# xudoong/EdgeVisionTransformer

Measured on AMD Instinct MI355X. Metric: images/sec DeiT-base/16-224 bs=512 @1/2/4/8 GPU; % bf16 MFMA roofline, higher is better.
Workload: dtype bf16; 1 GPU; deit_base/16-224 forward, bs=512 per GPU, bf16; model=deit_base, global_batch=512, per_gpu_batch=512, seq_len=197, parallelism=dp1, gemm_variant=automatic, lanes=1

## Files before the change

edgevisiontransformer_amd/_lib.py:

```python
from __future__ import annotations

import ctypes
import os
import threading

import torch

_HERE = os.path.dirname(os.path.abspath(__file__))
LIB_PATH = os.environ.get("EVT_LIB", os.path.join(_HERE, "libevt_hip.so"))

EVT_OK = 0
EVT_EINVAL = -22
EVT_ENOMEM = -12
EVT_EHIP = -5
EVT_ENODEV = -19
DTYPE = {"f32": 0, "fp32": 0, "float32": 0, "bf16": 1, "bfloat16": 1, "mx8": 2}

EPI_BIAS, EPI_GELU, EPI_RESID, EPI_POS, EPI_OUT_F32 = 1, 2, 4, 8, 16
EPI_LNIN, EPI_RESLN, EPI_STATS, EPI_GELU_ERF = 32, 64, 128, 256
EPI_OUT_MX8 = 512
PROF_ROLES = ("patchify", "patch_embed", "qkv", "attention", "out_proj", "fc1", "fc2", "head",
              "(unused)", "t2t_unfold", "t2t_kqv", "t2t_performer", "merge", "attn_sublayer",
              "mlp")
SWIN_MAX_STAGES = 8
# ... 163 lines not shown

class evt_attn_args(ctypes.Structure):
    _fields_ = [("n_maps", ctypes.c_int32), ("blocks", ctypes.POINTER(ctypes.c_int32)),
                ("maps", ctypes.POINTER(ctypes.c_void_p)), ("queries", ctypes.c_int32)]


ATTN_CLS, ATTN_ALL = 0, 1
ATTENTION_SIGNATURES = {
    "evt_attn_map_shape": (_I, [_P, _I, _PI, _PI]),
    "evt_forward_attention": (_I, [_P, ctypes.POINTER(evt_image_args), _I,
                                   ctypes.POINTER(evt_features_args),
                                   ctypes.POINTER(evt_attn_args), _P]),
    "evt_attention_probs": (_I, [_I, _P, _I64, _I64, _I64, _I, _I, _I, _I, _I, _F, _I, _P, _P]),
}

_lib = None
_lock = threading.Lock()
_initialized_devices = set()


def load_library() -> ctypes.CDLL:
    global _lib
    with _lock:
        if _lib is None:
            if not os.path.exists(LIB_PATH):
                raise ImportError(
                    f"{LIB_PATH} not found: build it with `python -m edgevisiontransformer_amd.build`"
                    " (hipcc --offload-arch=gfx950). There is no CPU fallback.")
            lib = ctypes.CDLL(LIB_PATH, mode=ctypes.RTLD_GLOBAL)
            lenient = "EVT_LIB" in os.environ
            for name, (res, args) in {**SIGNATURES, **EXT_SIGNATURES, **FEATURE_SIGNATURES,
                                      **IMAGE_SIGNATURES, **PREPROCESS_SIGNATURES,
                                      **ATTENTION_SIGNATURES}.items():
                if lenient and not hasattr(lib, name):
                    continue
                fn = getattr(lib, name)
                fn.restype = res
                fn.argtypes = args
            _lib = lib
    return _lib


def last_error() -> str:
    return load_library().evt_last_error().decode(errors="replace")


def check(rc: int) -> None:
    if rc != EVT_OK:
# ... 44 lines not shown
```

edgevisiontransformer_amd/build.py:

```python
from __future__ import annotations

import os
import subprocess
import sys
from concurrent.futures import ThreadPoolExecutor

HERE = os.path.dirname(os.path.abspath(__file__))
CSRC = os.path.join(HERE, "csrc")
LAB = os.environ.get("EVT_LAB", "") not in ("", "0")
LIB = os.path.join(HERE, "libevt_hip_lab.so" if LAB else "libevt_hip.so")
OBJ = os.path.join(HERE, "build_obj_lab" if LAB else "build_obj")
SOURCES = ["gemm.hip", "attention.hip", "norm.hip", "t2t.hip", "swin.hip", "mx8.hip",
           "features.hip", "preprocess.hip", "attn_maps.hip", "capi.cpp"]
HEADERS = ["common.h", "evt_internal.h", os.path.join("..", "..", "include", "evt.h"),
           os.path.join("..", "..", "include", "evt_patchify.h"),
           os.path.join("..", "..", "include", "evt_features.h"),
           os.path.join("..", "..", "include", "evt_image.h"),
           os.path.join("..", "..", "include", "evt_preprocess.h"),
           os.path.join("..", "..", "include", "evt_attention_maps.h")]
ARCH = os.environ.get("EVT_ARCH", "gfx950")
FLAGS = ["-O3", "-std=c++17", "-fPIC", f"--offload-arch={ARCH}", "-Wno-unused-result",
         "-ffp-contract=on"]
if LAB:
    FLAGS += ["-DEVT_GEMM_LAB"] + ([f"-DEVT_QA_DBG={os.environ['EVT_QA_DBG']}"]
                                   if os.environ.get("EVT_QA_DBG") else [])
    FLAGS += os.environ.get("EVT_LAB_DEFS", "").split()


PER_FILE_FLAGS = {s: ["-mllvm", "-amdgpu-mfma-vgpr-form=true"]
                  for s in ("attention.hip", "swin.hip", "t2t.hip", "attn_maps.hip")}
PER_FILE_FLAGS["attention.hip"] = PER_FILE_FLAGS["attention.hip"] + ["-fno-honor-nans"]
PER_FILE_FLAGS["swin.hip"] = PER_FILE_FLAGS["swin.hip"] + ["-fno-honor-nans"]


# ... 50 lines not shown
```

edgevisiontransformer_amd/csrc/attention.hip:

```cpp
#include "common.h"
#include "evt_internal.h"

namespace evt {

namespace {

template <int NKT>
__device__ __forceinline__ float prescale_nonpositive(f32x4 (&s)[NKT], float scale_log2) {
  if (scale_log2 > 0.f) return scale_log2;
#pragma unroll
  for (int kt = 0; kt < NKT; ++kt) s[kt] = s[kt] * scale_log2;
  return 1.f;
}


template <int NKT, bool PLAIN_STORE>
__device__ __forceinline__ void attn_tile_bf16(const AttnParams& p, const EVT_LDS char* Ks,
                                               const EVT_LDS char* Vs, u32x4 qf0, u32x4 qf1,
                                               int qt, int b, int h, int lane) {
  constexpr int ROWB = 128;
  const int g = lane >> 4, c16 = lane & 15, sw = lane & 7;
  f32x4 s[NKT];
#pragma unroll
  for (int kt = 0; kt < NKT; ++kt) {
// ... 143 lines not shown
    permlane16_swap(a0, c0);
    permlane16_swap(a1, c1);
    x0[pr] = a0; x1[pr] = a1; y0[pr] = c0; y1[pr] = c1;
  }
  if (q < p.N) {
    bf16* op = (bf16*)p.out + ((int64_t)b * p.N + q) * p.ldo + h * 64 + 16 * (g & 1) + 8 * (g >> 1);
#pragma unroll
    for (int pr = 0; pr < 2; ++pr) {
      const u32x4 v = {x0[pr], x1[pr], y0[pr], y1[pr]};
      if (PLAIN_STORE) store_b128(op + 32 * pr, v);
      else store_b128_nt(op + 32 * pr, v);
    }
  }
}

template <int NKT, int WAVES, int NQW, bool NT = false, bool NTQ = NT>
__device__ __forceinline__ void attn_stage_bf16(const AttnParams& p, EVT_LDS char* Ks,
                                                EVT_LDS char* Vs, u32x4 (&qf)[NQW][2], int b,
                                                int h, int wave, int lane) {
  constexpr int NP = NKT * 16, ROWB = 128;
  const bf16* qkv = (const bf16*)p.qkv + b * p.sb + h * p.sh;
  const int g = lane >> 4, c16 = lane & 15;
#pragma unroll
  for (int i = 0; i < NQW; ++i) {
    const int qi = min((wave + WAVES * i) * 16 + c16, p.N - 1);
    const bf16* qrow = qkv + (int64_t)qi * p.ldq;
    if (NTQ) {
      qf[i][0] = __builtin_nontemporal_load((const u32x4*)(qrow + 8 * g));
      qf[i][1] = __builtin_nontemporal_load((const u32x4*)(qrow + 8 * (g + 4)));
    } else {
      qf[i][0] = *(const u32x4*)(qrow + 8 * g);
      qf[i][1] = *(const u32x4*)(qrow + 8 * (g + 4));
    }
  }
  const int srow = lane >> 3, sslot = lane & 7;
  for (int i = wave; i < NP / 8; i += WAVES) {
    const int row = i * 8 + srow;
    const int gr = min(row, p.N - 1);
    const bf16* rp = qkv + (int64_t)gr * p.ldq + ((sslot ^ srow) * 8);
    if (NT) {
      __builtin_amdgcn_global_load_lds(rp + p.ko, Ks + i * 8 * ROWB, 16, 0, 2);
      __builtin_amdgcn_global_load_lds(rp + p.vo, Vs + i * 8 * ROWB, 16, 0, 2);
    } else {
      glds16(rp + p.ko, Ks + i * 8 * ROWB);
      glds16(rp + p.vo, Vs + i * 8 * ROWB);
    }
  }
}

template <int NKT, int NTM = 0>
__global__ __launch_bounds__(256, (NKT == 13 || NKT == 12) ? 3 : 1) void attn_bf16_kernel(AttnParams p) {
  extern __shared__ __attribute__((aligned(16))) char smem[];
  constexpr int NP = NKT * 16, ROWB = 128;
  constexpr int NQW = (NP / 16 + 3) / 4;
  EVT_LDS char* Ks = (EVT_LDS char*)smem;
  EVT_LDS char* Vs = Ks + NP * ROWB;
  const int tid = threadIdx.x, lane = tid & 63, wave = tid >> 6;
  const int b = blockIdx.x / p.H, h = blockIdx.x - b * p.H;
  const int nqt = (p.N + 15) >> 4;
  u32x4 qf[NQW][2];
  attn_stage_bf16<NKT, 4, NQW, (NTM == 1 || NTM == 2 || NTM == 4 || NTM == 5), (NTM == 1 || NTM == 4)>(
      p, Ks, Vs, qf, b, h, wave, lane);
  wait_vmcnt0();
  __syncthreads();
#pragma unroll
  for (int it = 0; it < NQW; ++it) {
    const int qt = wave + 4 * it;
    if (qt >= nqt) break;
    attn_tile_bf16<NKT, !(NTM == 1 || NTM == 3 || NTM == 5)>(p, Ks, Vs, qf[it][0], qf[it][1], qt, b, h, lane);
  }
}

#ifndef ATTN_F32_WAVES
#define ATTN_F32_WAVES 8
#endif

template <int NKT>
__global__ __launch_bounds__(64 * ATTN_F32_WAVES) void attn_f32_kernel(AttnParams p) {
  extern __shared__ __attribute__((aligned(16))) char smem[];
// ... 335 lines not shown
    hipLaunchKernelGGL((attn_gen_f32_kernel<NKT, 2>), dim3(p.B * p.H), dim3(256), 0, s, p);
  return hipGetLastError();
}

hipError_t attention_gen_launch(int dtype, const AttnParams& p, hipStream_t s) {
  if (p.N <= 64) return launch_gen<4>(dtype, p, s);
  if (p.N <= 128) return launch_gen<8>(dtype, p, s);
  if (p.N <= 208) return launch_gen<13>(dtype, p, s);
  return launch_gen<16>(dtype, p, s);
}

template <int NKT>
hipError_t launch_nkt(int dtype, const AttnParams& p, hipStream_t s) {
  const int rowb = dtype == DT_BF16 ? 128 : 256;
  const size_t lds = 2 * (size_t)NKT * 16 * rowb;
  if (dtype == DT_BF16)
    hipLaunchKernelGGL((attn_bf16_kernel<NKT, 5>), dim3(p.B * p.H), dim3(256), lds, s, p);
  else if constexpr (NKT % 2 == 0)
    hipLaunchKernelGGL(attn_f32_kernel<NKT>, dim3(p.B * p.H), dim3(64 * ATTN_F32_WAVES), lds, s, p);
  else
    return hipErrorInvalidValue;
  return hipGetLastError();
}


constexpr int LONG_KB = 64;
constexpr int LONG_NKT = LONG_KB / 16;

template <bool FAST>
__device__ __forceinline__ float online_softmax(f32x4 (&s)[LONG_NKT], float& m, float& l, float c) {
  float m0 = fmaxf(fmaxf(s[0][0], s[0][1]), s[0][2]), m1 = fmaxf(fmaxf(s[0][3], s[1][0]), s[1][1]);
// ... 391 lines not shown
}

bool g_attr_set = false;

void set_lds_attrs() {
  if (g_attr_set) return;
  g_attr_set = true;
  (void)hipFuncSetAttribute((const void*)attn_f32_kernel<14>, hipFuncAttributeMaxDynamicSharedMemorySize,
                      2 * 14 * 16 * 256);
  (void)hipFuncSetAttribute((const void*)attn_f32_kernel<16>, hipFuncAttributeMaxDynamicSharedMemorySize,
                      2 * 16 * 16 * 256);
}

}

hipError_t attention_launch(int dtype, const AttnParams& p_in, hipStream_t s) {
  if (p_in.B <= 0) return hipSuccess;
  if (p_in.N <= 0 || p_in.N > EVT_ATTN_MAX_TOKENS || p_in.H <= 0 || p_in.hd <= 0 || p_in.hd > 128)
    return hipErrorInvalidValue;
  if (p_in.N > 256 && p_in.q8) return hipErrorInvalidValue;
  if (p_in.N > 256 && !(p_in.scale_log2 > 0.f && p_in.scale_log2 < INFINITY)) return hipErrorInvalidValue;
  AttnParams p = p_in;
  const bool strided = p.sb || p.sh || p.ko || p.vo;
  if (strided) {
    if (dtype != DT_BF16 || p.hd != 64 || p.q8 || p.sb % 8 || p.sh % 8 || p.ldq % 8 || p.ko % 8 ||
        p.vo % 8 || p.ldq < 64 || p.ko < 0 || p.vo < 0 || p.sb < 0 || p.sh < 0)
      return hipErrorInvalidValue;
  } else {
    p.sb = (int64_t)p.N * p.ldq;
    p.sh = 64;
    p.ko = p.H * 64;
    p.vo = 2 * p.H * 64;
// ... 17 lines not shown
```

edgevisiontransformer_amd/csrc/capi.cpp:

```cpp
#include <hip/hip_runtime.h>

#include <algorithm>
#include <cmath>
#include <cstdio>
#include <cstdlib>
#include <cstring>
#include <functional>
#include <string>
#include <type_traits>
#include <vector>

#include "../../include/evt.h"
#include "evt_internal.h"

using namespace evt;

namespace {

thread_local std::string g_err;

int fail(int code, const std::string& msg) {
  g_err = msg;
  return code;
}
// ... 105 lines not shown
  float* su = nullptr;
  void* kqvb = nullptr;
  void* pout = nullptr;
  float* tstats = nullptr;
  void* zrow = nullptr;
  float* part = nullptr;
  void* apatch = nullptr;
  void* x = nullptr;
  void* xm = nullptr;
  float* sx = nullptr;
  float* sm = nullptr;
  void* qkv = nullptr;
  void* o = nullptr;
  void* hbuf = nullptr;
  size_t hbuf_bytes = 0;
  void* hh = nullptr;
  void* sk = nullptr;
  void* pooled = nullptr;
  void* qa = nullptr;
  uint32_t* sa = nullptr;
  void* qh = nullptr;
  uint32_t* shd = nullptr;
  float* lnst = nullptr;
  int qa_ld = 0, qh_ld = 0;
};
static_assert(std::is_trivially_copyable<Workspace>::value, "raw pointers and integers only");

struct evt_model : ModelCore {
  Workspace ws;
  int max_batch = 0;
  std::vector<void*> allocs;
  int hm_layers = 0;
  hipGraph_t graph = nullptr;
  hipGraphExec_t graph_exec = nullptr;
  bool prof = false;
  std::vector<hipEvent_t> prof_ev;
  std::vector<int> prof_role;
  mutable std::vector<double> prof_gflop, prof_gbytes;
  std::vector<evt_model*> lanes;
  std::vector<hipStream_t> lane_s;
  std::vector<char> lane_own;
  std::vector<hipEvent_t> lane_ev;
  bool is_lane = false;
  int no_balance = 0;
};

namespace {
// ... 195 lines not shown
size_t workspace_bytes(const evt_vit_desc* d, const Shape& sh, int B) {
  const bool mx8 = d->dtype == EVT_DTYPE_MX8;
  const size_t es = elem_size(mx8 ? DT_BF16 : d->dtype);
  const size_t rows = (size_t)B * sh.T;
  const size_t hb = std::max(rows * sh.max_ffn_st, (size_t)B * sh.P * sh.pdst) * es;
  size_t extra = 0;
  if (mx8) {
    const size_t qa = std::max(round_up(sh.D, 128), round_up(sh.max_inner, 128));
    int maxffn = 0;
    for (int i = 0; i < d->depth; ++i) maxffn = std::max(maxffn, (int)d->ffn[i]);
    const size_t qh = round_up(maxffn, 128);
    extra = rows * (qa + qa / 32 + qh + qh / 32 + 2 * sizeof(float)) + 5 * 256;
  }
  return 2 * rows * sh.D * es + 2 * rows * stats_slots(sh.D) * 2 * sizeof(float) +
         rows * 3 * sh.max_inner * es +
         rows * sh.max_inner * es + hb + (size_t)B * sh.head_st * es + 9 * 256 + extra;
}

struct DenseCall {
  int flags = 0;
  const void* A = nullptr;
  int64_t lda = 0;
  void* C = nullptr;
  int64_t ldc = 0;
  int M = 0, N = 0;
  const void* resid = nullptr;
  int64_t ldr = 0;
  const float* pos = nullptr;
  int64_t ldp = 0;
  int P = 0;
  const float* stats_in = nullptr;
  const float* rstats = nullptr;
  const float* rgamma = nullptr;
  const float* rbeta = nullptr;
  float* stats_out = nullptr;
  int ln_width = 0;
  int stats_step = 1;
  int slot_width = 0;
};

void dense_work(const evt_model* m, const DenseW& w, const DenseCall& c) {
  if (!m->prof) return;
  const double es = (double)elem_size(m->dtype);
  const double M = c.M, K = w.K, N = std::min(c.N, w.N);
  const int width = c.ln_width ? c.ln_width : m->D;
  const double slot_row = (double)stats_slots(c.slot_width ? c.slot_width : width) * 8.0;
  double bytes = M * K * es + K * N * es + M * N * ((c.flags & EPI_OUT_F32) ? 4.0 : es) + 8.0 * N;
  if (c.flags & EPI_RESID) bytes += M * N * es;
  if (c.flags & EPI_LNIN) bytes += M * slot_row;
  if (c.flags & EPI_RESLN) bytes += M * slot_row + 8.0 * N;
  if (c.flags & EPI_STATS) bytes += M * slot_row;
  if (c.flags & EPI_POS) bytes += (double)(c.P + 1) * N * 4.0;
  prof_work(m, 2.0 * M * K * N, bytes);
}

GemmParams dense_params(const evt_model* m, const DenseW& w, const DenseCall& c) {
  GemmParams p{};
  p.A = c.A;
  p.lda = c.lda;
// ... 15 lines not shown
  if (p.vec_ok && c.ldc % 8 == 0 && c.ldr % 8 == 0 && c.ldp % 8 == 0 &&
      (((uintptr_t)c.C | (uintptr_t)c.resid) & 15) == 0)
    p.vec_ok = 2;
  p.colsum = w.colsum;
  p.no_balance = m->no_balance;
  p.stats_in = c.stats_in;
  p.rstats = c.rstats;
  p.rgamma = c.rgamma;
  p.rbeta = c.rbeta;
  p.stats_out = c.stats_out;
  const int width = c.ln_width ? c.ln_width : m->D;
  p.inv_d = 1.0f / (float)width;
  p.eps = m->eps;
  p.nslots = stats_slots(c.slot_width ? c.slot_width : width);
  p.stats_step = c.stats_step;
  gemm_sk_bind(m->ws.sk, p);
  return p;
}

int dense(const evt_model* m, const DenseW& w, const DenseCall& c, hipStream_t s) {
  dense_work(m, w, c);
  const GemmParams p = dense_params(m, w, c);
  EVT_HIP(gemm_launch(m->dtype, c.flags, p, s), "dense");
  return EVT_OK;
}

int feat_export(evt_model* m, const void* x, int64_t ldx, int64_t row_step, float* out, bool norm,
                int rows, int D, hipStream_t s) {
  ProfScope ps(m, EVT_PROF_HEAD, s);
  prof_work(m, 0.0, (double)rows * D * (elem_size(m->dtype) + 4.0));
// ... 68 lines not shown
  }
  const size_t rows = (size_t)B * m->sh.T;
  const size_t xb = (rows * m->D + PAD_K) * es, ob = (rows * m->sh.max_inner + PAD_K) * es;
  EVT_RC(dev_alloc(m, &m->ws.x, xb));
  EVT_RC(dev_alloc(m, &m->ws.xm, xb));
  const size_t stats_bytes = rows * stats_slots(m->D) * 2 * sizeof(float);
  EVT_RC(dev_alloc(m, (void**)&m->ws.sx, stats_bytes));
  EVT_RC(dev_alloc(m, (void**)&m->ws.sm, stats_bytes));
  EVT_RC(dev_alloc(m, &m->ws.qkv, rows * 3 * m->sh.max_inner * es));
  EVT_RC(dev_alloc(m, &m->ws.o, ob));
  EVT_HIP(hipMemsetAsync(m->ws.x, 0, xb, s), "memset x");
  EVT_HIP(hipMemsetAsync(m->ws.xm, 0, xb, s), "memset xm");
  EVT_HIP(hipMemsetAsync(m->ws.o, 0, ob, s), "memset o");
  EVT_RC(dev_alloc(m, &m->ws.hbuf, hbuf_bytes));
  m->ws.hbuf_bytes = hbuf_bytes;
  return EVT_OK;
}

int dense_head(const evt_model* m, const DenseW& w, const DenseCall& c, hipStream_t s) {
  const int tiles = ((c.M + GEMM_BM - 1) / GEMM_BM) * (w.npad / GEMM_BN);
  int S = 1;
  while (S < 8 && tiles * S * 2 <= device_cus() && w.kpad % (S * 2 * PAD_K) == 0) S *= 2;
  const size_t part = (size_t)S * std::max(c.M, m->max_batch) * w.npad * sizeof(float);
  if (S < 2 || !m->ws.hbuf || part > m->ws.hbuf_bytes ||
      (c.flags & ~(EPI_BIAS | EPI_GELU | EPI_OUT_F32)))
    return dense(m, w, c, s);
  dense_work(m, w, c);
  GemmParams p{};
  p.A = c.A; p.lda = c.lda; p.W = w.w; p.ldw = w.kpad; p.C = c.C; p.ldc = c.ldc;
  p.M = c.M; p.N = c.N; p.K = w.kpad; p.ntiles = w.npad / GEMM_BN; p.bias = w.b;
  EVT_HIP(gemm_splitk_launch(m->dtype, c.flags, p, S, (float*)m->ws.hbuf, s), "dense (split-K)");
  return EVT_OK;
}

int run_encoder(evt_model* m, ForwardCall& call) {
  const int B = call.B, D = m->D, T = m->sh.T, rows = B * T;
  hipStream_t s = call.s;
  const float log2e = 1.4426950408889634f;
  m->hm_layers = 0;
  int block = 0;
  for (const Layer& L : m->layers) {
    const float scale_log2 = log2e / std::sqrt((float)L.hd);
    bool hm = false;
    {
      ProfScope ps(m, EVT_PROF_QKV, s);
      DenseCall c;
      c.flags = EPI_LNIN | EPI_BIAS;
      c.A = m->ws.x; c.lda = D; c.C = m->ws.qkv; c.ldc = 3 * L.inner; c.M = rows; c.N = 3 * L.inner;
      c.stats_in = m->ws.sx;
      if (L.hd == 64 && m->headmajor) {
        DenseCall h = c;
        h.flags |= EPI_HM;
        h.ldc = 64;
        h.P = T;
// ... 2 lines not shown
          hm = true;
          ++m->hm_layers;
        }
      }
      EVT_RC(dense(m, L.qkv, c, s));
    }
    AttnParams ap{m->ws.qkv, 3 * L.inner, m->ws.o, L.inner, T, L.heads, B, scale_log2};
    ap.hd = L.hd;
    if (hm) {
      ap.ldq = 64;
      ap.sb = (int64_t)L.heads * 3 * T * 64;
      ap.sh = (int64_t)3 * T * 64;
      ap.ko = T * 64;
      ap.vo = 2 * T * 64;
    }
    {
      ProfScope ps(m, EVT_PROF_ATTENTION, s);
      prof_work(m, 4.0 * B * L.heads * (double)T * T * L.hd,
                (double)rows * 4 * L.inner * elem_size(m->dtype));
      EVT_HIP(attention_launch(m->dtype, ap, s), "attention");
    }
    EVT_RC(attn_map(m, call, block, ap));
    DenseCall co;
    co.flags = m->standard ? (EPI_BIAS | EPI_RESID | EPI_STATS)
                           : (EPI_BIAS | EPI_RESID | EPI_RESLN | EPI_STATS);
    co.A = m->ws.o; co.lda = L.inner; co.C = m->ws.xm; co.ldc = D; co.M = rows; co.N = D;
    co.resid = m->ws.x; co.ldr = D; co.rstats = m->ws.sx; co.rgamma = L.ln1_g; co.rbeta = L.ln1_b;
    co.stats_out = m->ws.sm;
    DenseCall c1;
    c1.flags = EPI_LNIN | EPI_BIAS | (m->standard ? EPI_GELU_ERF : EPI_GELU);
    c1.A = m->ws.xm; c1.lda = D; c1.C = m->ws.hbuf; c1.ldc = L.ffn_st; c1.M = rows; c1.N = L.ffn_st;
    c1.stats_in = m->ws.sm;
    {
      ProfScope ps(m, EVT_PROF_OUT_PROJ, s);
      EVT_RC(dense(m, L.out, co, s));
    }
    {
      ProfScope ps(m, EVT_PROF_FC1, s);
      EVT_RC(dense(m, L.fc1, c1, s));
    }
    {
      ProfScope ps(m, EVT_PROF_FC2, s);
      DenseCall c;
      c.flags = m->standard ? (EPI_BIAS | EPI_RESID | EPI_STATS)
                            : (EPI_BIAS | EPI_RESID | EPI_RESLN | EPI_STATS);
      c.A = m->ws.hbuf; c.lda = L.ffn_st; c.C = m->ws.x; c.ldc = D; c.M = rows; c.N = D;
      c.resid = m->ws.xm; c.ldr = D; c.rstats = m->ws.sm; c.rgamma = L.ln2_g; c.rbeta = L.ln2_b;
      c.stats_out = m->ws.sx;
      EVT_RC(dense(m, L.fc2, c, s));
    }
    EVT_RC(feat_tap(m, call, block++, D, rows, D));
  }
  return EVT_OK;
}

int run_encoder_mx8(evt_model* m, ForwardCall& call) {
  const int B = call.B, D = m->D, T = m->sh.T, rows = B * T;
  hipStream_t s = call.s;
  const float log2e = 1.4426950408889634f;
  const int dpad = (int)round_up(D, 128);
  for (const Layer& L : m->layers) {
    EVT_HIP(ln_mx8_launch(m->ws.x, rows, D, dpad, L.ln1_g, L.ln1_b, m->eps, m->ws.lnst, m->ws.qa,
                          m->ws.sa, s),
            "ln1 mx8");
// ... 86 lines not shown
  const size_t t3 = (size_t)ts.grid[2] * ts.grid[2];
  return (size_t)B * std::max({t1 * round_up(ts.din[0], PAD_K), t2 * ts.din[1], t3 * ts.din[1]});
}

size_t t2t_unfold_stat_floats(const T2TShape& ts, int B) {
  const size_t t1 = (size_t)ts.grid[0] * ts.grid[0], t2 = (size_t)ts.grid[1] * ts.grid[1];
  return (size_t)B * std::max(t1 * stats_slots(ts.din[0]), t2 * stats_slots(ts.din[1])) * 2;
}

size_t t2t_workspace_bytes(const evt_t2t_desc* d, const T2TShape& ts, int B) {
  const size_t es = elem_size(d->dtype);
  const size_t rows = (size_t)B * ts.enc.T, t1 = (size_t)B * ts.grid[0] * ts.grid[0];
  return t2t_unfold_elems(ts, B) * es + t2t_unfold_stat_floats(ts, B) * 4 + t1 * 4 * 64 * es +
         performer_part_floats(B, ts.grid[0] * ts.grid[0]) * 4 + 2 * rows * d->dim * es +
         2 * rows * stats_slots(d->dim) * 2 * 4 + rows * 4 * ts.enc.max_inner * es +
         rows * ts.enc.max_ffn_st * es + t1 * 2 * 4 + 256;
}

struct SwinGeo {
  int ns = 0;
  int C[EVT_SWIN_MAX_STAGES], Cst[EVT_SWIN_MAX_STAGES], R[EVT_SWIN_MAX_STAGES];
  int mlp[EVT_SWIN_MAX_STAGES], mst[EVT_SWIN_MAX_STAGES];
  int w[EVT_SWIN_MAX_STAGES];
  int pd = 0, pdst = 0;
};

int validate_swin(const evt_swin_desc* d, SwinGeo* g) {
  if (!d) return fail(EVT_EINVAL, "desc is NULL");
  if (d->dtype != EVT_DTYPE_F32 && d->dtype != EVT_DTYPE_BF16)
    return fail(EVT_EINVAL, "dtype must be EVT_DTYPE_F32 or EVT_DTYPE_BF16");
  if (d->num_stages < 1 || d->num_stages > EVT_SWIN_MAX_STAGES)
// ... 157 lines not shown
  hipStream_t s = call.s;
  EVT_HIP(hipEventRecord(m->lane_ev[0], s), "lanes fork");
  for (int i = 0; i < k; ++i)
    EVT_HIP(hipStreamWaitEvent(m->lane_s[i], m->lane_ev[0], 0), "lane fork wait");
  for (int i = 0; i < k; ++i) {
    const int b0 = (int)((int64_t)B * i / k), b1 = (int)((int64_t)B * (i + 1) / k);
    if (b1 > b0) {
      ForwardCall lane = call.slice(b0, b1, m->img_elems, m->num_classes, m->lane_s[i]);
      EVT_RC(run_family(m->lanes[i], lane));
    }
    EVT_HIP(hipEventRecord(m->lane_ev[1 + i], m->lane_s[i]), "lane done");
  }
  for (int i = 0; i < k; ++i)
    EVT_HIP(hipStreamWaitEvent(s, m->lane_ev[1 + i], 0), "lanes join");
  m->hm_layers = m->lanes[0]->hm_layers;
  return EVT_OK;
}

static int check_batch(const evt_model* m, int B) {
  if (B <= 0 || B > m->max_batch)
    return fail(EVT_EINVAL, "batch must be in [1, max_batch=" + std::to_string(m->max_batch) + "]");
  return EVT_OK;
}

static int forward(evt_model* m, ForwardCall& call, bool use_lanes) {
  EVT_RC(check_batch(m, call.B));
  if (use_lanes && !m->lanes.empty() && !m->prof && call.B >= (int)m->lanes.size())
    return lanes_forward(m, call);
  return run_family(m, call);
}
// ... 425 lines not shown
    launches[r] = 0;
  }
  for (size_t i = 0; i < m->prof_role.size(); ++i) {
    EVT_HIP(hipEventSynchronize(m->prof_ev[2 * i + 1]), "profile sync");
    float ms = 0.f;
    EVT_HIP(hipEventElapsedTime(&ms, m->prof_ev[2 * i], m->prof_ev[2 * i + 1]), "profile read");
    us[m->prof_role[i]] += 1000.f * ms;
    launches[m->prof_role[i]] += 1;
  }
  return EVT_OK;
}

int evt_model_qkv_layout(const evt_model* m, int* headmajor_layers) {
  if (!m || !headmajor_layers) return fail(EVT_EINVAL, "null argument");
  *headmajor_layers = m->hm_layers;
  return EVT_OK;
}

int evt_model_set_lanes(evt_model* m, int lanes, void* stream) {
  if (!m) return fail(EVT_EINVAL, "model is NULL");
  if (m->is_lane) return fail(EVT_EINVAL, "the model is a lane of another model");
  if (lanes < 1 || lanes > 4) return fail(EVT_EINVAL, "lanes must be in [1, 4]");
  if (m->graph) return fail(EVT_EINVAL, "set the lanes before evt_graph_capture");
  (void)hipDeviceSynchronize();
  release_lanes(m);
  if (lanes == 1) return EVT_OK;
  hipStream_t s = (hipStream_t)stream;
  const int per = (m->max_batch + lanes - 1) / lanes;
  auto run = [&]() -> int {
    for (int i = 0; i < lanes; ++i) {
// ... 1245 lines not shown
```

edgevisiontransformer_amd/csrc/evt_internal.h:

```cpp
#pragma once
#include <hip/hip_runtime.h>
#include <stddef.h>
#include <stdint.h>

namespace evt {

enum Dtype : int { DT_F32 = 0, DT_BF16 = 1 };

struct ImgAffine {
  float scale[4], shift[4];
};

enum : int {
  EPI_BIAS = 1,
  EPI_GELU = 2,
  EPI_RESID = 4,
  EPI_POS = 8,
  EPI_OUT_F32 = 16,
  EPI_LNIN = 32,
  EPI_RESLN = 64,
  EPI_STATS = 128,
  EPI_GELU_ERF = 256,
  EPI_OUT_MX8 = 512,
  EPI_GATHER = 1024,
// ... 10 lines not shown
  const float* bias;
  const void* resid; int64_t ldr;
  const float* pos;  int64_t ldp;
  int P;
  int vec_ok;
  const float* colsum;
  const float* stats_in;
  const float* rstats;
  const float* rgamma;
  const float* rbeta;
  float* stats_out;
  float inv_d;
  float eps;
  int nslots;
  int stats_step;
  int gR, gC;
  float g_inv_rr, g_inv_r;
  int gmode, gOW;
  const void* gzero;
  int* sk_flags;
  float* sk_part;
  int ks_chunk;
  int64_t ks_stride;
  int xgroups;
  int no_balance;
};
constexpr int GEMM_BM = 128;
constexpr int GEMM_BN = 128;
constexpr int PACK_N = 256;
constexpr int PAD_K = 64;
// ... 18 lines not shown

struct AttnParams {
  const void* qkv; int64_t ldq;
  void* out;       int64_t ldo;
  int N;
  int H;
  int B;
  float scale_log2;
  uint8_t* q8 = nullptr;
  uint32_t* s8 = nullptr;
  int64_t ldq8 = 0;
  int rows8 = 0;
  int hd = 64;
  int64_t sb = 0, sh = 0;
  int ko = 0, vo = 0;
};
hipError_t attention_launch(int dtype, const AttnParams& p, hipStream_t s);
hipError_t attn_probs_launch(int dtype, const AttnParams& p, int nq, float* out, hipStream_t s);


hipError_t layernorm_launch(int dtype, const float* x, int64_t ldx, void* y, int64_t ldy,
                            const float* gamma, const float* beta, int rows, int D, float eps,
                            hipStream_t s);

hipError_t export_rows_launch(int dtype, const void* x, int64_t ldx, int64_t row_step, float* out,
                              const float* gamma, const float* beta, int rows, int D, float eps,
                              hipStream_t s);

__host__ __device__ inline int stats_slots(int D) { return 2 * ((D + 255) / 256); }

hipError_t patchify_launch(int dtype, const float* img, int B, int C, int HW, int ps, void* out,
                           void* x, const float* cls, const float* pos, int D, float* stats,
// ... 159 lines not shown
```

edgevisiontransformer_amd/csrc/gemm.hip:

```cpp
#include <type_traits>

#include "common.h"
#include "evt_internal.h"

namespace evt {

namespace {

constexpr int ROWB = 128;
constexpr int TILE_BYTES = GEMM_BM * ROWB;
constexpr int STAGE_BYTES = 2 * TILE_BYTES;

template <typename T> struct Mma;
template <> struct Mma<bf16> {
  static __device__ __forceinline__ void run(const u32x4& a, const u32x4& b, f32x4& c) {
    c = __builtin_amdgcn_mfma_f32_16x16x32_bf16(__builtin_bit_cast(bf16x8, a),
                                                __builtin_bit_cast(bf16x8, b), c, 0, 0, 0);
  }
};
template <> struct Mma<float> {
  static __device__ __forceinline__ void run(const u32x4& a, const u32x4& b, f32x4& c) {
    const f32x4 af = __builtin_bit_cast(f32x4, a), bf = __builtin_bit_cast(f32x4, b);
#pragma unroll
    for (int e = 0; e < 4; ++e) c = __builtin_amdgcn_mfma_f32_16x16x4f32(af[e], bf[e], c, 0, 0, 0);
// ... 39 lines not shown
                                           int row_lo, int lane, int slot) {
  typedef typename std::conditional<(FL & EPI_OUT_F32) != 0, float, T>::type TO;
  constexpr bool interior = INTERIOR;
  const int sub = lane >> 5, c = lane & 31;
  const bool col_ok = interior || n < p.N;
  const bool full = interior || (p.vec_ok && n + 4 <= p.N);
  f32x4 bias4 = f32x4{0.f, 0.f, 0.f, 0.f}, cs4 = bias4, g4 = bias4, b4 = bias4;
  if (col_ok) {
    if (FL & EPI_BIAS) bias4 = col4(p.bias, n, p.N, full);
    if (FL & EPI_LNIN) cs4 = col4(p.colsum, n, p.N, full);
    if (FL & EPI_RESLN) {
      g4 = col4(p.rgamma, n, p.N, full);
      b4 = col4(p.rbeta, n, p.N, full);
    }
  }
  float in_mu = 0.f, in_r = 0.f, rs_mu = 0.f, rs_r = 0.f;
  if (FL & (EPI_LNIN | EPI_RESLN)) {
    const int mr = m0 + row_lo + c;
    if (interior || mr < p.M) {
      if (FL & EPI_LNIN)
        ln_coef(p.stats_in, p.nslots, (int64_t)mr * (p.stats_step > 1 ? p.stats_step : 1), p.inv_d,
                p.eps, in_mu, in_r);
      if (FL & EPI_RESLN) ln_coef(p.rstats, p.nslots, mr, p.inv_d, p.eps, rs_mu, rs_r);
    }
  }
#pragma unroll
  for (int i = 0; i < 16; ++i) {
    if (i == 8) __builtin_amdgcn_sched_barrier(0);
    const int row = row_lo + 2 * i + sub;
    const int m = m0 + row;
    const bool ok = col_ok && (interior || m < p.M);
    f32x4 v = *(const EVT_LDS f32x4*)(stg + stg_off(row, c));
    int64_t orow = m;
    if (FL & EPI_LNIN) {
      const float mu = row_bcast(in_mu, 2 * i, sub), r = row_bcast(in_r, 2 * i, sub);
      if constexpr (std::is_same<T, float>::value) v = v * r + bias4;
      else v = v * r - cs4 * (r * mu) + bias4;
    } else if (FL & EPI_BIAS) {
// ... 47 lines not shown
#pragma unroll
    for (int j = 0; j < 8; ++j) {
      const f32x4 v = *(const EVT_LDS f32x4*)(src + j * 16);
      s1 += v[0] + v[2];
      s2 += v[1] + v[3];
    }
    s1 += __shfl_xor(s1, 32, 64);
    s2 += __shfl_xor(s2, 32, 64);
    const int m = m0 + row_lo + q;
    if (hf == 0 && (interior || m < p.M)) {
      int64_t orow = m;
      if (FL & EPI_POS) {
        const int img = m / p.P, t = m - img * p.P;
        orow = (int64_t)img * (p.P + 1) + 1 + t;
      }
      *(f32x2*)(p.stats_out + 2 * (p.nslots * orow + slot)) = f32x2{s1, s2};
    }
  }
}

template <int FL, bool INTERIOR>
__device__ __forceinline__ void epi_rows8_t(const GemmParams& p, EVT_LDS char* stg, int m0, int n,
                                            int row_lo, int lane, int slot) {
  constexpr bool interior = INTERIOR;
  const int q = lane >> 4, c8 = lane & 15;
  const bool col_ok = interior || n < p.N;
  const bool full = interior || n + 8 <= p.N;
  f32x4 bias4[2], cs4[2], g4[2], b4[2];
#pragma unroll
  for (int h = 0; h < 2; ++h) {
    bias4[h] = cs4[h] = g4[h] = b4[h] = f32x4{0.f, 0.f, 0.f, 0.f};
    const bool fh = interior || n + 4 * h + 4 <= p.N;
    if (col_ok) {
      if (FL & EPI_BIAS) bias4[h] = col4(p.bias, n + 4 * h, p.N, fh);
      if (FL & EPI_LNIN) cs4[h] = col4(p.colsum, n + 4 * h, p.N, fh);
      if (FL & EPI_RESLN) {
        g4[h] = col4(p.rgamma, n + 4 * h, p.N, fh);
        b4[h] = col4(p.rbeta, n + 4 * h, p.N, fh);
      }
    }
  }
  float in_mu = 0.f, in_r = 0.f, rs_mu = 0.f, rs_r = 0.f;
  if (FL & (EPI_LNIN | EPI_RESLN)) {
    const int mr = m0 + row_lo + (lane & 31);
    if (interior || mr < p.M) {
      if (FL & EPI_LNIN)
        ln_coef(p.stats_in, p.nslots, (int64_t)mr * (p.stats_step > 1 ? p.stats_step : 1), p.inv_d,
                p.eps, in_mu, in_r);
      if (FL & EPI_RESLN) ln_coef(p.rstats, p.nslots, mr, p.inv_d, p.eps, rs_mu, rs_r);
    }
  }
#pragma unroll
  for (int i = 0; i < 8; ++i) {
    if ((FL & EPI_RESID) ? (i & 1) == 0 && i > 0 : i == 4) __builtin_amdgcn_sched_barrier(0);
    const int row = row_lo + 4 * i + q;
    const int m = m0 + row;
    const bool ok = col_ok && (interior || m < p.M);
    const int src = (4 * i + q) * 4;
    f32x4 v[2];
    v[0] = *(const EVT_LDS f32x4*)(stg + stg_off(row, 2 * c8));
    v[1] = *(const EVT_LDS f32x4*)(stg + stg_off(row, 2 * c8 + 1));
    int64_t orow = m;
    if (FL & EPI_LNIN) {
      const float mu = __builtin_bit_cast(float, __builtin_amdgcn_ds_bpermute(src, __builtin_bit_cast(int, in_mu)));
// ... 70 lines not shown
#pragma unroll
    for (int j = 0; j < 4; ++j) {
      const f32x4 v = *(const EVT_LDS f32x4*)(src + j * 16);
      s1 += v[0] + v[2];
      s2 += v[1] + v[3];
    }
    s1 += __shfl_xor(s1, 32, 64);
    s2 += __shfl_xor(s2, 32, 64);
    const int m = m0 + row_lo + r;
    if (hf == 0 && (interior || m < p.M)) {
      int64_t orow = m;
      if (FL & EPI_POS) {
        const int img = m / p.P, t = m - img * p.P;
        orow = (int64_t)img * (p.P + 1) + 1 + t;
      }
      *(f32x2*)(p.stats_out + 2 * (p.nslots * orow + slot)) = f32x2{s1, s2};
    }
  }
}

template <typename T, int FL, bool ONLY8 = false>
__device__ __forceinline__ void epi_rows(const GemmParams& p, EVT_LDS char* stg, int m0, int n4,
                                         int n8, int row_lo, int lane, int slot, bool interior) {
  constexpr bool out16 = std::is_same<T, bf16>::value && !(FL & EPI_OUT_F32);
  if (out16 && (ONLY8 || p.vec_ok >= 2)) {
    if (interior) epi_rows8_t<FL, true>(p, stg, m0, n8, row_lo, lane, slot);
    else epi_rows8_t<FL, false>(p, stg, m0, n8, row_lo, lane, slot);
    return;
  }
  if constexpr (!(out16 && ONLY8)) {
    if (interior) epi_rows_t<T, FL, true>(p, stg, m0, n4, row_lo, lane, slot);
// ... 97 lines not shown
  epi_rows<T, FL>(p, stg, m0, n0 + (lane & 31) * 4, n0 + (lane & 15) * 8, wave * 32, lane,
                  n0 / 128, interior);
}

constexpr int BIG_BM = 256, BIG_BN = 256;
constexpr int BIG_TILE = BIG_BM * ROWB;
constexpr int BIG_STAGE = 2 * BIG_TILE;

thread_local int g_gemm_variant = 0;

int num_cus();

constexpr int64_t BIG_MAX_LD = ((int64_t)1 << 31) / (2 * 384) - 64;

bool use_big(const GemmParams& p, int flags) {
  if ((p.ntiles * GEMM_BN) % BIG_BN) return false;
  if (std::max(std::max(p.lda, p.ldw), std::max(p.ldc, p.resid ? p.ldr : (int64_t)0)) > BIG_MAX_LD)
    return false;
  if (!(flags & EPI_OUT_F32) && p.vec_ok < 2) return false;
  const int v = (g_gemm_variant == 31 || g_gemm_variant == 36) ? 0 : g_gemm_variant;
  if (v == 1) return false;
  if (v >= 2) return true;
  const int64_t G = num_cus();
  const int64_t t256 = (int64_t)((p.M + 255) / 256) * (p.ntiles * GEMM_BN / 256);
  const int64_t t128 = (int64_t)((p.M + 127) / 128) * p.ntiles;
  return (t256 + G - 1) / G <= 0.5 * (double)((t128 + G - 1) / G);
}

template <int FL>
__device__ __forceinline__ void big_epilogue(const GemmParams& p, char* smem, f32x4 (&acc)[4][8],
// ... 1813 lines not shown
constexpr bool pers_wide_fl(int fl) {
  return fl == (EPI_LNIN | EPI_BIAS) || fl == (EPI_LNIN | EPI_BIAS | EPI_GELU) ||
         fl == (EPI_LNIN | EPI_BIAS | EPI_GELU_ERF) || fl == (EPI_LNIN | EPI_BIAS | EPI_STATS) ||
         fl == (EPI_LNIN | EPI_BIAS | EPI_STATS | EPI_GATHER) ||
         fl == (EPI_BIAS | EPI_RESID | EPI_RESLN | EPI_STATS);
}
bool pers_wide(const GemmParams& p, int flags) {
  return (flags & (EPI_LNIN | EPI_RESLN)) && p.nslots > 8;
}

bool use_pers(const GemmParams& p, int flags) {
  const int v = g_gemm_variant;
  if (v != 0 && v != 9 && v != 16 && v != 31 && v != 36 && !gemm_lab_pers_variant(v))
    return false;
  if ((v == 13 || v == 15) && (flags & EPI_POS)) return false;
  if (p.N % 8 || p.vec_ok < 2) return false;
  if ((flags & (EPI_LNIN | EPI_RESLN)) && (p.nslots > 12 || p.nslots % 2 || p.stats_step > 1))
    return false;
  if (pers_wide(p, flags) && (!pers_wide_fl(flags) || p.K / 64 < PERS_WIDE_MIN_NK || v == 16 ||
                              gemm_lab_pers_variant(v)))
    return false;
  if ((flags & EPI_POS) && (!p.resid || p.ldr % 8 || p.P <= 0 || p.M >= (1 << 22))) return false;
  return true;
}

int pers_xgroups(int ntiles, int G, int total) {
  if (G != 256 || total <= G) return 1;
  return (ntiles % 2 == 0 && ntiles / 2 >= 3) ? 2 : 1;
}

template <int FL>
// ... 46 lines not shown
    hipLaunchKernelGGL((gemm_pers_kernel<FL, 7, false>), dim3(G), dim3(512), 0, s, q, total);
  else if (g_gemm_variant == 18)
    hipLaunchKernelGGL((gemm_pers_kernel<(FL & ~(EPI_GELU | EPI_GELU_ERF)), 0, false>), dim3(G),
                       dim3(512), 0, s, q, total);
#endif
  else if (p.N % BIG_BN == 0)
    hipLaunchKernelGGL((gemm_pers_kernel<FL, 0, false>), dim3(G), dim3(512), 0, s, q, total);
  else
    hipLaunchKernelGGL((gemm_pers_kernel<FL>), dim3(G), dim3(512), 0, s, q, total);
  return hipGetLastError();
}

bool use_p384(const GemmParams& p, int flags) {
  const int v = g_gemm_variant;
  if ((v != 0 && v != 30) || p.N % 384 || p.vec_ok < 2 || p.K < 64) return false;
  if (std::max(std::max(p.lda, p.ldw), std::max(p.ldc, p.resid ? p.ldr : (int64_t)0)) > BIG_MAX_LD)
    return false;
  if ((flags & (EPI_LNIN | EPI_RESLN)) && (p.nslots > 8 || p.nslots % 2 || p.stats_step > 1))
    return false;
  if ((flags & EPI_STATS) && 3 * (p.N / 384) > p.nslots) return false;
  return v == 30;
}

template <int FL>
hipError_t launch_p384(const GemmParams& p, hipStream_t s) {
  GemmParams q = p;
  q.ntiles = p.N / 384;
  const int total = ((p.M + 127) / 128) * q.ntiles;
  int G = min(total, num_cus());
  if (G >= 8 && total > G) G &= ~7;
// ... 266 lines not shown
```

edgevisiontransformer_amd/modeling/models/_handle.py:

```python
from __future__ import annotations

import ctypes
from typing import List, Optional, Union

import numpy as np
import torch

from ... import _lib
from ...images import Uint8Images


def _to_device_image(img, device):
    if isinstance(img, Uint8Images):
        return img.to(device), img.is_numpy
    if isinstance(img, np.ndarray):
        return torch.from_numpy(np.ascontiguousarray(img, dtype=np.float32)).to(device), True
    if not isinstance(img, torch.Tensor):
        raise TypeError("img must be a torch.Tensor or numpy.ndarray")
    if img.dtype != torch.float32:
        img = img.float()
    if img.device != device:
        img = img.to(device)
    return img.contiguous(), False

# ... 46 lines not shown
        with torch.cuda.device(self.device):
            _lib.check(getattr(lib, self._C_CREATE)(ctypes.byref(desc), ptrs, n, self._stream(),
                                                    ctypes.byref(out)))
            self._handle = out.value
            self._max_batch = max_batch
            self._lane_streams = _lib.set_lanes(
                self._handle, self._lanes if self._lanes is not None
                else _lib.default_lanes(self.dtype, max_batch, **self._DEFAULT_LANES_KW),
                self.device)

    def lanes(self) -> int:
        out = ctypes.c_int()
        _lib.check(_lib.load_library().evt_model_lanes(self._ptr(), ctypes.byref(out)))
        return out.value

    def workspace_bytes(self, batch: int) -> int:
        out = ctypes.c_size_t()
        _lib.check(getattr(_lib.load_library(), self._C_QUERY_WORKSPACE)(
            ctypes.byref(self._desc(batch)), batch, ctypes.byref(out)))
        return out.value

    def close(self) -> None:
        if getattr(self, "_handle", None):
            _lib.load_library().evt_model_destroy(self._ptr())
            self._handle = None

    def __del__(self):
        try:
            self.close()
        except Exception:
# ... 62 lines not shown
```

include/evt.h:

```cpp
#ifndef EVT_H_
#define EVT_H_

#include <stddef.h>
#include <stdint.h>

#ifdef __cplusplus
extern "C" {
#endif

#define EVT_OK 0
#define EVT_EINVAL (-22)
#define EVT_ENOMEM (-12)
#define EVT_EHIP (-5)
#define EVT_ENODEV (-19)

#define EVT_DTYPE_F32 0
#define EVT_DTYPE_BF16 1
#define EVT_DTYPE_MX8 2

typedef struct evt_vit_desc {
  int32_t image_size;
  int32_t patch_size;
  int32_t in_chans;
  int32_t num_classes;
// ... 216 lines not shown


int evt_set_gemm_variant(int variant);

int evt_model_qkv_layout(const evt_model* m, int* headmajor_layers);

#ifdef __cplusplus
}
#endif

#include "evt_patchify.h"
#include "evt_features.h"
#include "evt_image.h"
#include "evt_preprocess.h"
#include "evt_attention_maps.h"

#endif
```

Measured before the change: 29660 images/s.

## Compute only CLS token rows in final transformer block when features unused

In the last encoder block, attention computes only the first query tile, and the out-proj, fc1 and fc2 GEMMs run on just the CLS row of each image via strided leading dimensions and stats steps. A separate small hidden buffer is allocated for this tail. Full computation is kept when token features or last-block taps are requested. Strided small-M GEMMs are forced onto the non-persistent path, which may use the hardware less efficiently.

```diff
diff --git a/edgevisiontransformer_amd/_lib.py b/edgevisiontransformer_amd/_lib.py
--- a/edgevisiontransformer_amd/_lib.py
+++ b/edgevisiontransformer_amd/_lib.py
@@ -201,6 +201,10 @@
     "evt_attention_probs": (_I, [_I, _P, _I64, _I64, _I64, _I, _I, _I, _I, _I, _F, _I, _P, _P]),
 }
 
+TAIL_SIGNATURES = {
+    "evt_model_tail_mode": (_I, [_P, _PI]),
+}
+
 _lib = None
 _lock = threading.Lock()
 _initialized_devices = set()
@@ -218,7 +222,7 @@
             lenient = "EVT_LIB" in os.environ
             for name, (res, args) in {**SIGNATURES, **EXT_SIGNATURES, **FEATURE_SIGNATURES,
                                       **IMAGE_SIGNATURES, **PREPROCESS_SIGNATURES,
-                                      **ATTENTION_SIGNATURES}.items():
+                                      **ATTENTION_SIGNATURES, **TAIL_SIGNATURES}.items():
                 if lenient and not hasattr(lib, name):
                     continue
                 fn = getattr(lib, name)
diff --git a/edgevisiontransformer_amd/build.py b/edgevisiontransformer_amd/build.py
--- a/edgevisiontransformer_amd/build.py
+++ b/edgevisiontransformer_amd/build.py
@@ -17,7 +17,8 @@
            os.path.join("..", "..", "include", "evt_features.h"),
            os.path.join("..", "..", "include", "evt_image.h"),
            os.path.join("..", "..", "include", "evt_preprocess.h"),
-           os.path.join("..", "..", "include", "evt_attention_maps.h")]
+           os.path.join("..", "..", "include", "evt_attention_maps.h"),
+           os.path.join("..", "..", "include", "evt_tail.h")]
 ARCH = os.environ.get("EVT_ARCH", "gfx950")
 FLAGS = ["-O3", "-std=c++17", "-fPIC", f"--offload-arch={ARCH}", "-Wno-unused-result",
          "-ffp-contract=on"]
diff --git a/edgevisiontransformer_amd/csrc/attention.hip b/edgevisiontransformer_amd/csrc/attention.hip
--- a/edgevisiontransformer_amd/csrc/attention.hip
+++ b/edgevisiontransformer_amd/csrc/attention.hip
@@ -181,7 +181,7 @@
   }
 }
 
-template <int NKT, int WAVES, int NQW, bool NT = false, bool NTQ = NT>
+template <int NKT, int WAVES, int NQW, bool NT = false, bool NTQ = NT, bool Q0 = false>
 __device__ __forceinline__ void attn_stage_bf16(const AttnParams& p, EVT_LDS char* Ks,
                                                 EVT_LDS char* Vs, u32x4 (&qf)[NQW][2], int b,
                                                 int h, int wave, int lane) {
@@ -190,6 +190,7 @@
   const int g = lane >> 4, c16 = lane & 15;
 #pragma unroll
   for (int i = 0; i < NQW; ++i) {
+    if (Q0 && wave != 0) break;
     const int qi = min((wave + WAVES * i) * 16 + c16, p.N - 1);
     const bf16* qrow = qkv + (int64_t)qi * p.ldq;
     if (NTQ) {
@@ -215,21 +216,22 @@
   }
 }
 
-template <int NKT, int NTM = 0>
+template <int NKT, int NTM = 0, bool CLS = false>
 __global__ __launch_bounds__(256, (NKT == 13 || NKT == 12) ? 3 : 1) void attn_bf16_kernel(AttnParams p) {
   extern __shared__ __attribute__((aligned(16))) char smem[];
   constexpr int NP = NKT * 16, ROWB = 128;
-  constexpr int NQW = (NP / 16 + 3) / 4;
+  constexpr int NQW = CLS ? 1 : (NP / 16 + 3) / 4;
   EVT_LDS char* Ks = (EVT_LDS char*)smem;
   EVT_LDS char* Vs = Ks + NP * ROWB;
   const int tid = threadIdx.x, lane = tid & 63, wave = tid >> 6;
   const int b = blockIdx.x / p.H, h = blockIdx.x - b * p.H;
   const int nqt = (p.N + 15) >> 4;
   u32x4 qf[NQW][2];
-  attn_stage_bf16<NKT, 4, NQW, (NTM == 1 || NTM == 2 || NTM == 4 || NTM == 5), (NTM == 1 || NTM == 4)>(
+  attn_stage_bf16<NKT, 4, NQW, (NTM == 1 || NTM == 2 || NTM == 4 || NTM == 5), (NTM == 1 || NTM == 4), CLS>(
       p, Ks, Vs, qf, b, h, wave, lane);
   wait_vmcnt0();
   __syncthreads();
+  if (CLS && wave != 0) return;
 #pragma unroll
   for (int it = 0; it < NQW; ++it) {
     const int qt = wave + 4 * it;
@@ -595,7 +597,9 @@
 hipError_t launch_nkt(int dtype, const AttnParams& p, hipStream_t s) {
   const int rowb = dtype == DT_BF16 ? 128 : 256;
   const size_t lds = 2 * (size_t)NKT * 16 * rowb;
-  if (dtype == DT_BF16)
+  if (dtype == DT_BF16 && p.cls_only)
+    hipLaunchKernelGGL((attn_bf16_kernel<NKT, 5, true>), dim3(p.B * p.H), dim3(256), lds, s, p);
+  else if (dtype == DT_BF16)
     hipLaunchKernelGGL((attn_bf16_kernel<NKT, 5>), dim3(p.B * p.H), dim3(256), lds, s, p);
   else if constexpr (NKT % 2 == 0)
     hipLaunchKernelGGL(attn_f32_kernel<NKT>, dim3(p.B * p.H), dim3(64 * ATTN_F32_WAVES), lds, s, p);
@@ -1017,8 +1021,13 @@
 
 }
 
+bool attention_cls_ok(int dtype, const AttnParams& p) {
+  return dtype == DT_BF16 && p.hd == 64 && p.N <= 256 && !p.q8;
+}
+
 hipError_t attention_launch(int dtype, const AttnParams& p_in, hipStream_t s) {
   if (p_in.B <= 0) return hipSuccess;
+  if (p_in.cls_only && !attention_cls_ok(dtype, p_in)) return hipErrorInvalidValue;
   if (p_in.N <= 0 || p_in.N > EVT_ATTN_MAX_TOKENS || p_in.H <= 0 || p_in.hd <= 0 || p_in.hd > 128)
     return hipErrorInvalidValue;
   if (p_in.N > 256 && p_in.q8) return hipErrorInvalidValue;
diff --git a/edgevisiontransformer_amd/csrc/capi.cpp b/edgevisiontransformer_amd/csrc/capi.cpp
--- a/edgevisiontransformer_amd/csrc/capi.cpp
+++ b/edgevisiontransformer_amd/csrc/capi.cpp
@@ -143,6 +143,7 @@
   void* o = nullptr;
   void* hbuf = nullptr;
   size_t hbuf_bytes = 0;
+  void* hc = nullptr;
   void* hh = nullptr;
   void* sk = nullptr;
   void* pooled = nullptr;
@@ -160,6 +161,7 @@
   int max_batch = 0;
   std::vector<void*> allocs;
   int hm_layers = 0;
+  int tail_mode = 0;
   hipGraph_t graph = nullptr;
   hipGraphExec_t graph_exec = nullptr;
   bool prof = false;
@@ -385,7 +387,8 @@
   }
   return 2 * rows * sh.D * es + 2 * rows * stats_slots(sh.D) * 2 * sizeof(float) +
          rows * 3 * sh.max_inner * es +
-         rows * sh.max_inner * es + hb + (size_t)B * sh.head_st * es + 9 * 256 + extra;
+         rows * sh.max_inner * es + hb + (size_t)B * sh.max_ffn_st * es +
+         (size_t)B * sh.head_st * es + 10 * 256 + extra;
 }
 
 struct DenseCall {
@@ -408,12 +411,15 @@
   int ln_width = 0;
   int stats_step = 1;
   int slot_width = 0;
+  int rs_step = 1;
+  bool force_nt = false;
+  int work_M = 0;
 };
 
 void dense_work(const evt_model* m, const DenseW& w, const DenseCall& c) {
-  if (!m->prof) return;
+  if (!m->prof || c.work_M < 0) return;
   const double es = (double)elem_size(m->dtype);
-  const double M = c.M, K = w.K, N = std::min(c.N, w.N);
+  const double M = c.work_M ? c.work_M : c.M, K = w.K, N = std::min(c.N, w.N);
   const int width = c.ln_width ? c.ln_width : m->D;
   const double slot_row = (double)stats_slots(c.slot_width ? c.slot_width : width) * 8.0;
   double bytes = M * K * es + K * N * es + M * N * ((c.flags & EPI_OUT_F32) ? 4.0 : es) + 8.0 * N;
@@ -459,6 +465,8 @@
   p.eps = m->eps;
   p.nslots = stats_slots(c.slot_width ? c.slot_width : width);
   p.stats_step = c.stats_step;
+  p.rs_step = c.rs_step;
+  p.force_nt = c.force_nt;
   gemm_sk_bind(m->ws.sk, p);
   return p;
 }
@@ -557,6 +565,7 @@
   EVT_HIP(hipMemsetAsync(m->ws.o, 0, ob, s), "memset o");
   EVT_RC(dev_alloc(m, &m->ws.hbuf, hbuf_bytes));
   m->ws.hbuf_bytes = hbuf_bytes;
+  if (!m->mx8) EVT_RC(dev_alloc(m, &m->ws.hc, (size_t)B * m->sh.max_ffn_st * es));
   return EVT_OK;
 }
 
@@ -581,6 +590,7 @@
   hipStream_t s = call.s;
   const float log2e = 1.4426950408889634f;
   m->hm_layers = 0;
+  m->tail_mode = 0;
   int block = 0;
   for (const Layer& L : m->layers) {
     const float scale_log2 = log2e / std::sqrt((float)L.hd);
@@ -613,11 +623,20 @@
       ap.ko = T * 64;
       ap.vo = 2 * T * 64;
     }
+    const bool last = block + 1 == (int)m->layers.size();
+    bool full = !last;
+    if (last && call.feat) {
+      const evt_features_args* a = call.feat;
+      full = a->tokens || (a->n_taps > 0 && a->tap_blocks[a->n_taps - 1] == block);
+    }
+    if (last) m->tail_mode = full ? 3 : 1;
     {
       ProfScope ps(m, EVT_PROF_ATTENTION, s);
       prof_work(m, 4.0 * B * L.heads * (double)T * T * L.hd,
                 (double)rows * 4 * L.inner * elem_size(m->dtype));
-      EVT_HIP(attention_launch(m->dtype, ap, s), "attention");
+      AttnParams aq = ap;
+      aq.cls_only = !full && attention_cls_ok(m->dtype, ap);
+      EVT_HIP(attention_launch(m->dtype, aq, s), "attention");
     }
     EVT_RC(attn_map(m, call, block, ap));
     DenseCall co;
@@ -630,23 +649,37 @@
     c1.flags = EPI_LNIN | EPI_BIAS | (m->standard ? EPI_GELU_ERF : EPI_GELU);
     c1.A = m->ws.xm; c1.lda = D; c1.C = m->ws.hbuf; c1.ldc = L.ffn_st; c1.M = rows; c1.N = L.ffn_st;
     c1.stats_in = m->ws.sm;
+    DenseCall c2;
+    c2.flags = co.flags;
+    c2.A = m->ws.hbuf; c2.lda = L.ffn_st; c2.C = m->ws.x; c2.ldc = D; c2.M = rows; c2.N = D;
+    c2.resid = m->ws.xm; c2.ldr = D; c2.rstats = m->ws.sm; c2.rgamma = L.ln2_g; c2.rbeta = L.ln2_b;
+    c2.stats_out = m->ws.sx;
+    auto tail = [&](DenseCall c) {
+      c.M = B;
+      if (c.A == m->ws.hbuf) c.A = m->ws.hc;
+      else c.lda *= T;
+      if (c.C == m->ws.hbuf) c.C = m->ws.hc;
+      else c.ldc *= T;
+      c.ldr *= T;
+      c.stats_step = c.rs_step = T;
+      c.force_nt = true;
+      c.work_M = full ? -1 : rows;
+      return c;
+    };
     {
       ProfScope ps(m, EVT_PROF_OUT_PROJ, s);
-      EVT_RC(dense(m, L.out, co, s));
+      if (full) EVT_RC(dense(m, L.out, co, s));
+      if (last) EVT_RC(dense(m, L.out, tail(co), s));
     }
     {
       ProfScope ps(m, EVT_PROF_FC1, s);
-      EVT_RC(dense(m, L.fc1, c1, s));
+      if (full) EVT_RC(dense(m, L.fc1, c1, s));
+      if (last) EVT_RC(dense(m, L.fc1, tail(c1), s));
     }
     {
       ProfScope ps(m, EVT_PROF_FC2, s);
-      DenseCall c;
-      c.flags = m->standard ? (EPI_BIAS | EPI_RESID | EPI_STATS)
-                            : (EPI_BIAS | EPI_RESID | EPI_RESLN | EPI_STATS);
-      c.A = m->ws.hbuf; c.lda = L.ffn_st; c.C = m->ws.x; c.ldc = D; c.M = rows; c.N = D;
-      c.resid = m->ws.xm; c.ldr = D; c.rstats = m->ws.sm; c.rgamma = L.ln2_g; c.rbeta = L.ln2_b;
-      c.stats_out = m->ws.sx;
-      EVT_RC(dense(m, L.fc2, c, s));
+      if (full) EVT_RC(dense(m, L.fc2, c2, s));
+      if (last) EVT_RC(dense(m, L.fc2, tail(c2), s));
     }
     EVT_RC(feat_tap(m, call, block++, D, rows, D));
   }
@@ -763,7 +796,8 @@
   return t2t_unfold_elems(ts, B) * es + t2t_unfold_stat_floats(ts, B) * 4 + t1 * 4 * 64 * es +
          performer_part_floats(B, ts.grid[0] * ts.grid[0]) * 4 + 2 * rows * d->dim * es +
          2 * rows * stats_slots(d->dim) * 2 * 4 + rows * 4 * ts.enc.max_inner * es +
-         rows * ts.enc.max_ffn_st * es + t1 * 2 * 4 + 256;
+         rows * ts.enc.max_ffn_st * es + (size_t)B * ts.enc.max_ffn_st * es +
+         t1 * 2 * 4 + 2 * 256;
 }
 
 struct SwinGeo {
@@ -951,6 +985,7 @@
   for (int i = 0; i < k; ++i)
     EVT_HIP(hipStreamWaitEvent(s, m->lane_ev[1 + i], 0), "lanes join");
   m->hm_layers = m->lanes[0]->hm_layers;
+  m->tail_mode = m->lanes[0]->tail_mode;
   return EVT_OK;
 }
 
@@ -1406,6 +1441,12 @@
 int evt_model_qkv_layout(const evt_model* m, int* headmajor_layers) {
   if (!m || !headmajor_layers) return fail(EVT_EINVAL, "null argument");
   *headmajor_layers = m->hm_layers;
+  return EVT_OK;
+}
+
+int evt_model_tail_mode(const evt_model* m, int* mode) {
+  if (!m || !mode) return fail(EVT_EINVAL, "null argument");
+  *mode = m->tail_mode;
   return EVT_OK;
 }
 
diff --git a/edgevisiontransformer_amd/csrc/evt_internal.h b/edgevisiontransformer_amd/csrc/evt_internal.h
--- a/edgevisiontransformer_amd/csrc/evt_internal.h
+++ b/edgevisiontransformer_amd/csrc/evt_internal.h
@@ -48,6 +48,8 @@
   float eps;
   int nslots;
   int stats_step;
+  int rs_step;
+  int force_nt;
   int gR, gC;
   float g_inv_rr, g_inv_r;
   int gmode, gOW;
@@ -96,8 +98,10 @@
   int hd = 64;
   int64_t sb = 0, sh = 0;
   int ko = 0, vo = 0;
+  int cls_only = 0;
 };
 hipError_t attention_launch(int dtype, const AttnParams& p, hipStream_t s);
+bool attention_cls_ok(int dtype, const AttnParams& p);
 hipError_t attn_probs_launch(int dtype, const AttnParams& p, int nq, float* out, hipStream_t s);
 
 
diff --git a/edgevisiontransformer_amd/csrc/gemm.hip b/edgevisiontransformer_amd/csrc/gemm.hip
--- a/edgevisiontransformer_amd/csrc/gemm.hip
+++ b/edgevisiontransformer_amd/csrc/gemm.hip
@@ -77,6 +77,7 @@
       b4 = col4(p.rbeta, n, p.N, full);
     }
   }
+  const int64_t rs_step = p.rs_step > 1 ? p.rs_step : 1;
   float in_mu = 0.f, in_r = 0.f, rs_mu = 0.f, rs_r = 0.f;
   if (FL & (EPI_LNIN | EPI_RESLN)) {
     const int mr = m0 + row_lo + c;
@@ -84,7 +85,7 @@
       if (FL & EPI_LNIN)
         ln_coef(p.stats_in, p.nslots, (int64_t)mr * (p.stats_step > 1 ? p.stats_step : 1), p.inv_d,
                 p.eps, in_mu, in_r);
-      if (FL & EPI_RESLN) ln_coef(p.rstats, p.nslots, mr, p.inv_d, p.eps, rs_mu, rs_r);
+      if (FL & EPI_RESLN) ln_coef(p.rstats, p.nslots, (int64_t)mr * rs_step, p.inv_d, p.eps, rs_mu, rs_r);
     }
   }
 #pragma unroll
@@ -162,7 +163,7 @@
         const int img = m / p.P, t = m - img * p.P;
         orow = (int64_t)img * (p.P + 1) + 1 + t;
       }
-      *(f32x2*)(p.stats_out + 2 * (p.nslots * orow + slot)) = f32x2{s1, s2};
+      *(f32x2*)(p.stats_out + 2 * (p.nslots * orow * rs_step + slot)) = f32x2{s1, s2};
     }
   }
 }
@@ -188,6 +189,7 @@
       }
     }
   }
+  const int64_t rs_step = p.rs_step > 1 ? p.rs_step : 1;
   float in_mu = 0.f, in_r = 0.f, rs_mu = 0.f, rs_r = 0.f;
   if (FL & (EPI_LNIN | EPI_RESLN)) {
     const int mr = m0 + row_lo + (lane & 31);
@@ -195,7 +197,7 @@
       if (FL & EPI_LNIN)
         ln_coef(p.stats_in, p.nslots, (int64_t)mr * (p.stats_step > 1 ? p.stats_step : 1), p.inv_d,
                 p.eps, in_mu, in_r);
-      if (FL & EPI_RESLN) ln_coef(p.rstats, p.nslots, mr, p.inv_d, p.eps, rs_mu, rs_r);
+      if (FL & EPI_RESLN) ln_coef(p.rstats, p.nslots, (int64_t)mr * rs_step, p.inv_d, p.eps, rs_mu, rs_r);
     }
   }
 #pragma unroll
@@ -296,7 +298,7 @@
         const int img = m / p.P, t = m - img * p.P;
         orow = (int64_t)img * (p.P + 1) + 1 + t;
       }
-      *(f32x2*)(p.stats_out + 2 * (p.nslots * orow + slot)) = f32x2{s1, s2};
+      *(f32x2*)(p.stats_out + 2 * (p.nslots * orow * rs_step + slot)) = f32x2{s1, s2};
     }
   }
 }
@@ -424,6 +426,7 @@
 constexpr int64_t BIG_MAX_LD = ((int64_t)1 << 31) / (2 * 384) - 64;
 
 bool use_big(const GemmParams& p, int flags) {
+  if (p.force_nt || p.rs_step > 1) return false;
   if ((p.ntiles * GEMM_BN) % BIG_BN) return false;
   if (std::max(std::max(p.lda, p.ldw), std::max(p.ldc, p.resid ? p.ldr : (int64_t)0)) > BIG_MAX_LD)
     return false;
@@ -2267,7 +2270,7 @@
   if (v != 0 && v != 9 && v != 16 && v != 31 && v != 36 && !gemm_lab_pers_variant(v))
     return false;
   if ((v == 13 || v == 15) && (flags & EPI_POS)) return false;
-  if (p.N % 8 || p.vec_ok < 2) return false;
+  if (p.N % 8 || p.vec_ok < 2 || p.force_nt || p.rs_step > 1) return false;
   if ((flags & (EPI_LNIN | EPI_RESLN)) && (p.nslots > 12 || p.nslots % 2 || p.stats_step > 1))
     return false;
   if (pers_wide(p, flags) && (!pers_wide_fl(flags) || p.K / 64 < PERS_WIDE_MIN_NK || v == 16 ||
@@ -2344,6 +2347,7 @@
 bool use_p384(const GemmParams& p, int flags) {
   const int v = g_gemm_variant;
   if ((v != 0 && v != 30) || p.N % 384 || p.vec_ok < 2 || p.K < 64) return false;
+  if (p.force_nt || p.rs_step > 1) return false;
   if (std::max(std::max(p.lda, p.ldw), std::max(p.ldc, p.resid ? p.ldr : (int64_t)0)) > BIG_MAX_LD)
     return false;
   if ((flags & (EPI_LNIN | EPI_RESLN)) && (p.nslots > 8 || p.nslots % 2 || p.stats_step > 1))
diff --git a/edgevisiontransformer_amd/modeling/models/_handle.py b/edgevisiontransformer_amd/modeling/models/_handle.py
--- a/edgevisiontransformer_amd/modeling/models/_handle.py
+++ b/edgevisiontransformer_amd/modeling/models/_handle.py
@@ -84,6 +84,11 @@
         _lib.check(_lib.load_library().evt_model_lanes(self._ptr(), ctypes.byref(out)))
         return out.value
 
+    def tail_mode(self) -> int:
+        out = ctypes.c_int()
+        _lib.check(_lib.load_library().evt_model_tail_mode(self._ptr(), ctypes.byref(out)))
+        return out.value
+
     def workspace_bytes(self, batch: int) -> int:
         out = ctypes.c_size_t()
         _lib.check(getattr(_lib.load_library(), self._C_QUERY_WORKSPACE)(
diff --git a/include/evt.h b/include/evt.h
--- a/include/evt.h
+++ b/include/evt.h
@@ -254,5 +254,6 @@
 #include "evt_image.h"
 #include "evt_preprocess.h"
 #include "evt_attention_maps.h"
+#include "evt_tail.h"
 
 #endif
diff --git a/include/evt_tail.h b/include/evt_tail.h
--- /dev/null
+++ b/include/evt_tail.h
@@ -0,0 +1,14 @@
+#ifndef EVT_TAIL_H_
+#define EVT_TAIL_H_
+#ifdef __cplusplus
+extern "C" {
+#endif
+
+struct evt_model;
+
+int evt_model_tail_mode(const struct evt_model* m, int* mode);
+
+#ifdef __cplusplus
+}
+#endif
+#endif
```

After: 31410 images/s (median of 6 runs). +5.9%, better.
